# XinMing0411/AC-VAE

Measured on AMD Instinct MI355X. Metric: train-step captions/s (and audio-sec/s) at B=32, 1/2/4/8 MI355X, higher is better.
Workload: dtype f32

## Files before the change

### acvae_amd/csrc/conv_wino.hip

```cpp
#include "mfma_tile.h"
#include "../../include/acvae_hip.h"
#include "conv.h"
#include "prof.h"
#include <type_traits>

namespace {
using namespace mfma;

constexpr int WN_THREADS = 256;
constexpr int WN_TILES = 32;
constexpr int WN_TN = 64;
constexpr int WN_SC = 66, WN_SR = 2 * WN_SC, WN_SQ = 276;
constexpr int WN_BCHUNK = 16 * 2 * 64;
constexpr int WN_MAXC = 2048;
#ifndef WN_PRIO_EDGE
#define WN_PRIO_EDGE 3
#endif
#ifndef WN_PF_DIST
#define WN_PF_DIST 64
#endif

constexpr int WN_RAWBUF = 4 * WN_SQ;
constexpr int WN_EX_F4 = 6 * 512;
constexpr int WN_LDS_F4 = WN_EX_F4 + 64;
static_assert(2 * WN_RAWBUF <= WN_LDS_F4 && 2 * WN_RAWBUF + 2 * WN_MAXC / 4 >= WN_LDS_F4, "exchange + sums overlay the window buffers (+ scale / shift)");

__device__ __forceinline__ void wino_tile(int row, int tw_shift, int& tyl, int& tx) {
  const int cell = (int)((0x1c0c081804141000ULL >> (8 * (row >> 2))) & 0xff) + (row & 3);
  if (tw_shift >= 4) {
    tyl = cell >> tw_shift;
    tx = cell & ((1 << tw_shift) - 1);
  } else {
    const int g = cell >> 4, l16 = cell & 15;
    tx = l16 & ((1 << tw_shift) - 1);
    tyl = g + 2 * (l16 >> tw_shift);
  }
}
__host__ __device__ __forceinline__ int wino_row_pitch(int tw_shift) {
  return tw_shift == 3 ? 12 : tw_shift == 2 ? 6 : (1 << tw_shift) + 1;
}

struct WinoParams {
  const float* X;
  const float* scale;
  const float* shift;
  const float* U;
  float* Y;
  float* partials;
  const float* rY;
  const float* rscale;
  const float* rshift;
  const float* rmean;
  const float* rinvstd;
  int N, H, W, C, Cout;
  int tw_shift;
  int R;
  int bpc;
  int w_shift;
  unsigned bpc_magic;
  int nn_shift;
  int bn_group;
};
__device__ __forceinline__ void wino_tile_of(const WinoParams& p, int t, int nm, int nn, int& bm, int& bn) {
  if (p.bn_group) {
    const int G = p.bn_group, per = nm * G;
    int grp = (int)__fdividef((float)t, (float)per);
    int rem = t - grp * per;
    if (rem < 0) { --grp; rem += per; } else if (rem >= per) { ++grp; rem -= per; }
    bm = rem >> (G >> 1);
    bn = grp * G + (rem & (G - 1));
  } else if (p.nn_shift >= 0) { bn = t & (nn - 1); bm = t >> p.nn_shift; }
  else { bn = t % nn; bm = t / nn; }
}
__device__ __forceinline__ int wino_xcd_tile(const WinoParams& p, int nm, int nn, int& bm, int& bn) {
  const int total = nm * nn;
  const int b = blockIdx.x + blockIdx.y * nm;
  const int q = total >> 3, r = total & 7;
  const int xcd = b & 7, idx = b >> 3;
  const int t = xcd * q + (xcd < r ? xcd : r) + idx;
  wino_tile_of(p, t, nm, nn, bm, bn);
  return t;
}

typedef float f32x2 __attribute__((ext_vector_type(2)));
#define WN_PK_SUB(d, a, b) "v_pk_add_f32 " d ", " a ", " b " neg_lo:[0,1] neg_hi:[0,1]\n\t"
#define WN_PK_ADD(d, a, b) "v_pk_add_f32 " d ", " a ", " b "\n\t"
__device__ __forceinline__ float4 f4sub(float4 a, float4 b) {
  f32x2 lo, hi;
  asm(WN_PK_SUB("%0", "%2", "%4") WN_PK_SUB("%1", "%3", "%5")
      : "=&v"(lo), "=&v"(hi) : "v"(f32x2{a.x, a.y}), "v"(f32x2{a.z, a.w}), "v"(f32x2{b.x, b.y}), "v"(f32x2{b.z, b.w}));
  return make_float4(lo[0], lo[1], hi[0], hi[1]);
}
__device__ __forceinline__ float4 f4add(float4 a, float4 b) {
  f32x2 lo, hi;
  asm(WN_PK_ADD("%0", "%2", "%4") WN_PK_ADD("%1", "%3", "%5")
      : "=&v"(lo), "=&v"(hi) : "v"(f32x2{a.x, a.y}), "v"(f32x2{a.z, a.w}), "v"(f32x2{b.x, b.y}), "v"(f32x2{b.z, b.w}));
  return make_float4(lo[0], lo[1], hi[0], hi[1]);
}
__device__ __forceinline__ void wino_htrans(const float4 (&t)[4], float4 (&v)[4]) {
  f32x2 o[8];
  asm(WN_PK_SUB("%0", "%8", "%12") WN_PK_SUB("%1", "%9", "%13")
      WN_PK_ADD("%2", "%10", "%12") WN_PK_ADD("%3", "%11", "%13")
      WN_PK_SUB("%4", "%12", "%10") WN_PK_SUB("%5", "%13", "%11")
      WN_PK_SUB("%6", "%10", "%14") WN_PK_SUB("%7", "%11", "%15")
      "s_nop 1"
      : "=&v"(o[0]), "=&v"(o[1]), "=&v"(o[2]), "=&v"(o[3]), "=&v"(o[4]), "=&v"(o[5]), "=&v"(o[6]), "=&v"(o[7])
      : "v"(f32x2{t[0].x, t[0].y}), "v"(f32x2{t[0].z, t[0].w}), "v"(f32x2{t[1].x, t[1].y}), "v"(f32x2{t[1].z, t[1].w}),
        "v"(f32x2{t[2].x, t[2].y}), "v"(f32x2{t[2].z, t[2].w}), "v"(f32x2{t[3].x, t[3].y}), "v"(f32x2{t[3].z, t[3].w}));
#pragma unroll
  for (int k = 0; k < 4; ++k) v[k] = make_float4(o[2 * k][0], o[2 * k][1], o[2 * k + 1][0], o[2 * k + 1][1]);
}
__device__ __forceinline__ void pk_sub_ip(float4& a, const float4& b) {
  f32x2 lo{a.x, a.y}, hi{a.z, a.w};
  asm(WN_PK_SUB("%0", "%0", "%2") WN_PK_SUB("%1", "%1", "%3") : "+v"(lo), "+v"(hi) : "v"(f32x2{b.x, b.y}), "v"(f32x2{b.z, b.w}));
  a = make_float4(lo[0], lo[1], hi[0], hi[1]);
}
__device__ __forceinline__ void pk_add_ip(float4& a, const float4& b) {
  f32x2 lo{a.x, a.y}, hi{a.z, a.w};
  asm(WN_PK_ADD("%0", "%0", "%2") WN_PK_ADD("%1", "%1", "%3") : "+v"(lo), "+v"(hi) : "v"(f32x2{b.x, b.y}), "v"(f32x2{b.z, b.w}));
  a = make_float4(lo[0], lo[1], hi[0], hi[1]);
}
__device__ __forceinline__ void wino_htrans_ip(float4 (&t)[4], float4 (&v)[4]) {
  f32x2 a0{t[0].x, t[0].y}, a1{t[0].z, t[0].w}, c0{t[2].x, t[2].y}, c1{t[2].z, t[2].w}, e0{t[3].x, t[3].y}, e1{t[3].z, t[3].w};
  f32x2 n0, n1;
  asm(WN_PK_SUB("%0", "%0", "%2") WN_PK_SUB("%1", "%1", "%3")
      WN_PK_ADD("%6", "%8", "%2") WN_PK_ADD("%7", "%9", "%3")
      WN_PK_SUB("%2", "%2", "%8") WN_PK_SUB("%3", "%3", "%9")
      WN_PK_SUB("%4", "%8", "%4") WN_PK_SUB("%5", "%9", "%5")
      "s_nop 1"
      : "+v"(a0), "+v"(a1), "+v"(c0), "+v"(c1), "+v"(e0), "+v"(e1), "=&v"(n0), "=&v"(n1)
      : "v"(f32x2{t[1].x, t[1].y}), "v"(f32x2{t[1].z, t[1].w}));
  v[0] = make_float4(a0[0], a0[1], a1[0], a1[1]);
  v[1] = make_float4(n0[0], n0[1], n1[0], n1[1]);
  v[2] = make_float4(c0[0], c0[1], c1[0], c1[1]);
  v[3] = make_float4(e0[0], e0[1], e1[0], e1[1]);
}
__device__ __forceinline__ void mfma4_first(f32x16& c, float4 a, float4 b) {
  const f32x16 z = {0.f, 0.f, 0.f, 0.f, 0.f, 0.f, 0.f, 0.f, 0.f, 0.f, 0.f, 0.f, 0.f, 0.f, 0.f, 0.f};
  c = __builtin_amdgcn_mfma_f32_32x32x2f32(a.x, b.x, z, 0, 0, 0);
  c = __builtin_amdgcn_mfma_f32_32x32x2f32(a.y, b.y, c, 0, 0, 0);
  c = __builtin_amdgcn_mfma_f32_32x32x2f32(a.z, b.z, c, 0, 0, 0);
  c = __builtin_amdgcn_mfma_f32_32x32x2f32(a.w, b.w, c, 0, 0, 0);
}
__device__ __forceinline__ void mfma4(f32x16& c, float4 a, float4 b) {
  c = __builtin_amdgcn_mfma_f32_32x32x2f32(a.x, b.x, c, 0, 0, 0);
  c = __builtin_amdgcn_mfma_f32_32x32x2f32(a.y, b.y, c, 0, 0, 0);
  c = __builtin_amdgcn_mfma_f32_32x32x2f32(a.z, b.z, c, 0, 0, 0);
  c = __builtin_amdgcn_mfma_f32_32x32x2f32(a.w, b.w, c, 0, 0, 0);
}

template <int XI, int MODE>
__device__ __forceinline__ void wino_epilogue(const WinoParams& p, const f32x16 (&acc)[8], float2* ex, float* red, int li, int h,
                                              int lane, int n, int ty0, int bm, int bn) {
  constexpr int ROW = XI >> 1, NH = XI & 1;
  constexpr int SET_OTHER = XI == 0 ? 0 : XI == 1 ? 1 : XI == 2 ? 4 : 5;
  constexpr int SET_OWN = XI == 1 ? 2 : XI == 2 ? 3 : -1;
  constexpr int SET_A = XI == 0 ? 1 : XI == 1 ? 0 : XI == 2 ? 1 : 2, SET_B = XI == 0 ? 3 : XI == 1 ? 4 : XI == 2 ? 5 : 4;
  constexpr bool STATS = MODE != 0;
  const int tid = XI * 64 + lane;
  const int H = p.H, W = p.W, Cout = p.Cout;
  const int cout = bn * WN_TN + NH * 32 + li;
  int yk[4], voff[4];
#pragma unroll
  for (int k = 0; k < 4; ++k) {
    int tyl, tx;
    wino_tile(8 * k + 4 * h, p.tw_shift, tyl, tx);
    yk[k] = 2 * (ty0 + tyl) + ROW;
    voff[k] = ((yk[k] * W + 2 * tx) * Cout + cout) * 4;
  }
  int dyj[4], soff[4];
#pragma unroll
  for (int j = 0; j < 4; ++j) {
    dyj[j] = p.tw_shift == 1 ? 4 * (j >> 1) : 0;
    const int dx = p.tw_shift == 1 ? 2 * (j & 1) : 2 * j;
    soff[j] = (dyj[j] * W + dx) * Cout * 4;
  }
  const int pix = Cout * 4;
  float2 yv[MODE == 2 ? 16 : 1];
  float rsc = 0.f, rsh = 0.f, rmu = 0.f, ris = 0.f;
  if (MODE == 2) {
    const __amdgpu_buffer_rsrc_t rrs = __builtin_amdgcn_make_buffer_rsrc(const_cast<float*>(p.rY) + (long)n * H * W * Cout, 0, H * W * Cout * 4, 0x00020000);
#pragma unroll
    for (int r = 0; r < 16; ++r) {
      yv[r].x = __uint_as_float(__builtin_amdgcn_raw_buffer_load_b32(rrs, voff[r >> 2], soff[r & 3], 0));
      yv[r].y = __uint_as_float(__builtin_amdgcn_raw_buffer_load_b32(rrs, voff[r >> 2], soff[r & 3] + pix, 0));
    }
    rsc = p.rscale[cout]; rsh = p.rshift[cout]; rmu = p.rmean[cout]; ris = p.rinvstd[cout];
  }
  float2 keep[16];
#pragma unroll
  for (int r = 0; r < 16; ++r) {
#pragma unroll
    for (int nh = 0; nh < 2; ++nh) {
      const float m0 = acc[0 + nh][r], m1 = acc[2 + nh][r], m2 = acc[4 + nh][r], m3 = acc[6 + nh][r];
      const float2 f = make_float2(m0 + m1 + m2, m1 - m2 - m3);
      if (nh == NH) {
        keep[r] = f;
        if (SET_OWN >= 0) ex[(SET_OWN * 16 + r) * 64 + lane] = f;
      } else {
        ex[(SET_OTHER * 16 + r) * 64 + lane] = f;
      }
    }
  }
  __syncthreads();
  const __amdgpu_buffer_rsrc_t yrs = __builtin_amdgcn_make_buffer_rsrc(p.Y + (long)n * H * W * Cout, 0, H * W * Cout * 4, 0x00020000);
  float s = 0.f, qq = 0.f;
#pragma unroll
  for (int r = 0; r < 16; ++r) {
    const int k = r >> 2, j = r & 3;
    const float2 a = ex[(SET_A * 16 + r) * 64 + lane], b = ex[(SET_B * 16 + r) * 64 + lane];
    const float o0 = ROW ? a.x - (b.x + keep[r].x) : (keep[r].x + a.x) + b.x, o1 = ROW ? a.y - (b.y + keep[r].y) : (keep[r].y + a.y) + b.y;
    __builtin_amdgcn_raw_buffer_store_b32(__float_as_uint(o0), yrs, voff[k], soff[j], 0);
    __builtin_amdgcn_raw_buffer_store_b32(__float_as_uint(o1), yrs, voff[k], soff[j] + pix, 0);
    if (MODE == 1) {
      const bool ok = yk[k] + dyj[j] < H;
      const float a0 = ok ? o0 : 0.f, a1 = ok ? o1 : 0.f;
      s += a0 + a1;
      qq += a0 * a0 + a1 * a1;
    }
    if (MODE == 2) {
      const bool ok = yk[k] + dyj[j] < H;
      const float g0 = (ok && yv[r].x * rsc + rsh > 0.f) ? o0 : 0.f, g1 = (ok && yv[r].y * rsc + rsh > 0.f) ? o1 : 0.f;
      s += g0; s += g1;
      qq += g0 * ((yv[r].x - rmu) * ris); qq += g1 * ((yv[r].y - rmu) * ris);
    }
  }
  if (STATS && p.partials) {
    s += __shfl_xor(s, 32, 64);
    qq += __shfl_xor(qq, 32, 64);
    if (h == 0) {
      red[(ROW * 2 + 0) * 64 + NH * 32 + li] = s;
      red[(ROW * 2 + 1) * 64 + NH * 32 + li] = qq;
    }
    __syncthreads();
    if (tid < WN_TN) {
      const float ts = red[(0 * 2 + 0) * 64 + tid] + red[(1 * 2 + 0) * 64 + tid], tq = red[(0 * 2 + 1) * 64 + tid] + red[(1 * 2 + 1) * 64 + tid];
      float* out = p.partials + (long)bm * 2 * p.Cout + bn * WN_TN + tid;
      out[0] = ts;
      out[p.Cout] = tq;
    }
  }
}

template <int XI, bool ACT, int STATS>
__device__ __forceinline__ void conv_wino_body(const WinoParams& p, float4* raw0, float4* raw1, float4* scsh) {
  __builtin_amdgcn_s_setprio(WN_PRIO_EDGE);
  const int tid = threadIdx.x, lane = tid & 63;
  const int li = lane & 31, h = lane >> 5;
  int bm, bn;
  const int tpos = wino_xcd_tile(p, gridDim.x, gridDim.y, bm, bn);
  const int RW = wino_row_pitch(p.tw_shift), R = p.R;
  const int n = p.bpc == 1 ? bm : (int)__umulhi((unsigned)bm, p.bpc_magic), ty0 = (bm - n * p.bpc) * R;
  const int H = p.H, W = p.W, C = p.C;

  const int nitems = ((2 * R + 2) << p.w_shift) * 4;
  const int q = tid & 3;
  for (int i = tid; i < (2 * R + 2) * 8; i += WN_THREADS) {
    const int ry = i >> 3, side = (i >> 2) & 1, qi = i & 3;
    const int rx = side ? W + 1 : 0;
    const int slot = qi * WN_SQ + (ry & 1) * WN_SR + (rx & 1) * WN_SC + (ry >> 1) * RW + (rx >> 1);
    raw0[slot] = make_float4(0.f, 0.f, 0.f, 0.f);
    raw1[slot] = make_float4(0.f, 0.f, 0.f, 0.f);
  }
  unsigned goff[4];
  int loff[4];
#pragma unroll
  for (int j = 0; j < 4; ++j) {
    const int e = tid + WN_THREADS * j;
    const bool lv = e < nitems;
    const int px = e >> 2;
    const int ry = px >> p.w_shift, x = px & (W - 1), rx = x + 1;
    const int y = 2 * ty0 - 1 + ry;
    const bool ok = lv && y >= 0 && y < H;
    goff[j] = ok ? (unsigned)((((long)(n * H + y) * W + x) * C) + q * 4) : 0u;
    const int slot = q * WN_SQ + (ry & 1) * WN_SR + (rx & 1) * WN_SC + (ry >> 1) * RW + (rx >> 1);
    if (lv && !ok) {
      raw0[slot] = make_float4(0.f, 0.f, 0.f, 0.f);
      raw1[slot] = make_float4(0.f, 0.f, 0.f, 0.f);
    }
    loff[j] = ok ? slot : WN_RAWBUF - 1 - (tid & 7);
  }
  float4 pv[4];
  auto issue_raw = [&](int st) {
#pragma unroll
    for (int j = 0; j < 4; ++j) pv[j] = *reinterpret_cast<const float4*>(p.X + goff[j] + st * 16);
  };
  auto stage_scsh = [&]() {
    if (ACT) {
      for (int i = tid; i < (C >> 2); i += WN_THREADS) {
        scsh[i] = *reinterpret_cast<const float4*>(p.scale + 4 * i);
        scsh[(C >> 2) + i] = *reinterpret_cast<const float4*>(p.shift + 4 * i);
      }
      __syncthreads();
    }
  };
  float4 sc = make_float4(1.f, 1.f, 1.f, 1.f), sh = make_float4(0.f, 0.f, 0.f, 0.f);
  auto read_scsh = [&](int st) {
    if (ACT) {
      sc = scsh[st * 4 + q];
      sh = scsh[(C >> 2) + st * 4 + q];
    }
  };
  auto put_raw_part = [&](float4* raw, int j0) {
#pragma unroll
    for (int j = j0; j < j0 + 2; ++j) {
      float4 v = pv[j];
      if (ACT) {
        v.x = fmaxf(v.x * sc.x + sh.x, 0.f); v.y = fmaxf(v.y * sc.y + sh.y, 0.f);
        v.z = fmaxf(v.z * sc.z + sh.z, 0.f); v.w = fmaxf(v.w * sc.w + sh.w, 0.f);
      }
      raw[loff[j]] = v;
    }
  };
  auto put_raw = [&](float4* raw) { put_raw_part(raw, 0); put_raw_part(raw, 2); };
  const int nchunk = C >> 3;
  const __amdgpu_buffer_rsrc_t urs = __builtin_amdgcn_make_buffer_rsrc(
      const_cast<float*>(p.U + ((long)bn * nchunk) * (WN_BCHUNK * 4)), 0, 0x7fffffff, 0x00020000);
  int tyl_a, tx_a;
  wino_tile(li, p.tw_shift, tyl_a, tx_a);
  const int abase = tyl_a * RW + tx_a;
  constexpr int RA = XI == 0 ? 0 : XI == 2 ? 2 : 1, RB = XI == 0 ? 2 : XI == 1 ? 2 : XI == 2 ? 1 : 3;
  const int rowa = (RA & 1) * WN_SR + (RA >> 1) * RW + abase, rowb = (RB & 1) * WN_SR + (RB >> 1) * RW + abase;
  const int bvoff = (h * 64 + li) * 16;
  auto load_b = [&](int c, int g) {
    typedef unsigned wn_v4u __attribute__((ext_vector_type(4)));
    const wn_v4u v = __builtin_amdgcn_raw_buffer_load_b128(urs, bvoff, c * (WN_BCHUNK * 16) + (XI * 4 + (g >> 1)) * 2048 + (g & 1) * 512, 0);
    return make_float4(__uint_as_float(v.x), __uint_as_float(v.y), __uint_as_float(v.z), __uint_as_float(v.w));
  };

  f32x16 acc[8];

  const int nstage = C >> 4;
  const float4* const aq0 = raw0 + h * WN_SQ;
  const float4* const aq1 = raw1 + h * WN_SQ;
  float4 va[4], vb[4], B[4];
  auto read_row = [&](const float4* rq, int row, float4 (&d)[4]) {
#pragma unroll
    for (int j = 0; j < 4; ++j) d[j] = rq[row + (j & 1) * WN_SC + (j >> 1)];
  };
  auto vertical = [&](float4 (&da)[4], float4 (&db)[4]) {
#pragma unroll
    for (int j = 0; j < 4; ++j) {
      if (XI == 1) pk_add_ip(da[j], db[j]); else pk_sub_ip(da[j], db[j]);
    }
  };

#pragma unroll
  for (int g = 0; g < 4; ++g) B[g] = load_b(0, g);
  issue_raw(0);
  stage_scsh();
  read_scsh(0);
  put_raw(raw0);
  issue_raw(nstage > 1 ? 1 : 0);
  __syncthreads();
  {
    float4 da[4], db[4];
    read_row(aq0, rowa, da);
    read_row(aq0, rowb, db);
    vertical(da, db);
    wino_htrans_ip(da, va);
  }
#define WN_SB() __builtin_amdgcn_sched_barrier(0)
  auto step = [&](int c, auto kk, auto first) {
    constexpr int K = decltype(kk)::value;
    constexpr bool FIRST = decltype(first)::value;
    auto mm = [&](f32x16& a_, float4 x_, float4 y_) { if (FIRST) mfma4_first(a_, x_, y_); else mfma4(a_, x_, y_); };
    constexpr int sub = K & 1, sp = K >> 1;
    float4 (&vc)[4] = sub ? vb : va;
    float4 (&vn)[4] = sub ? va : vb;
    const int st = c >> 1;
    float4* const rnxt = sp ? raw0 : raw1;
    const float4* const nq = sub ? (sp ? aq0 : aq1) : (sp ? aq1 : aq0) + 2 * WN_SQ;
    const int cn = c + 1 < nchunk ? c + 1 : c;
    float4 da[4], db[4];
    const int st1 = st + 1 < nstage ? st + 1 : nstage - 1, st2 = st + 2 < nstage ? st + 2 : nstage - 1;
    if (sub == 0) read_scsh(st1);
    WN_SB();
    mm(acc[0], vc[0], B[0]);
    WN_SB();
    B[0] = load_b(c, 4);
    if (sub == 0) put_raw_part(rnxt, 0);
    WN_SB();
    mm(acc[1], vc[0], B[1]);
    WN_SB();
    B[1] = load_b(c, 5);
    if (sub == 0) put_raw_part(rnxt, 2);
    WN_SB();
    mm(acc[2], vc[1], B[2]);
    WN_SB();
    B[2] = load_b(c, 6);
    if (sub == 0) issue_raw(st2);
    WN_SB();
    mm(acc[3], vc[1], B[3]);
    WN_SB();
    B[3] = load_b(c, 7);
    read_row(nq, rowa, da);
    WN_SB();
    mm(acc[4], vc[2], B[0]);
    WN_SB();
    B[0] = load_b(cn, 0);
    read_row(nq, rowb, db);
    WN_SB();
    mm(acc[5], vc[2], B[1]);
    WN_SB();
    B[1] = load_b(cn, 1);
    WN_SB();
    mm(acc[6], vc[3], B[2]);
    WN_SB();
    B[2] = load_b(cn, 2);
    vertical(da, db);
    WN_SB();
    mm(acc[7], vc[3], B[3]);
    WN_SB();
    B[3] = load_b(cn, 3);
    wino_htrans_ip(da, vn);
    WN_SB();
    if (sub == 0) __syncthreads();
  };
#undef WN_SB
  using std::integral_constant;
  using std::false_type;
  __builtin_amdgcn_s_setprio(0);
  step(0, integral_constant<int, 0>(), std::true_type());
  step(1, integral_constant<int, 1>(), false_type());
  if (2 < nchunk) {
    step(2, integral_constant<int, 2>(), false_type());
    step(3, integral_constant<int, 3>(), false_type());
  }
  for (int c = 4; c < nchunk; c += 4) {
    step(c, integral_constant<int, 0>(), false_type());
    step(c + 1, integral_constant<int, 1>(), false_type());
    if (c + 2 < nchunk) {
      step(c + 2, integral_constant<int, 2>(), false_type());
      step(c + 3, integral_constant<int, 3>(), false_type());
    }
  }
  __builtin_amdgcn_s_setprio(WN_PRIO_EDGE);
  __syncthreads();
  const int lane_e = (int)__builtin_amdgcn_mbcnt_hi(~0u, __builtin_amdgcn_mbcnt_lo(~0u, 0u));
  const int li_e = lane_e & 31, h_e = lane_e >> 5;
  const int tid_e = XI * 64 + lane_e;

  float pfv = 0.f;
  if (!ACT) {
    const int nn_ = (int)gridDim.y;
    const int t2 = tpos + WN_PF_DIST * ((int)gridDim.x * nn_ >= 8 * WN_PF_DIST ? 1 : 0);
    int bm2 = bm, bn2 = bn;
    if (t2 < (int)gridDim.x * nn_) wino_tile_of(p, t2, (int)gridDim.x, nn_, bm2, bn2);
    const int n2 = p.bpc == 1 ? bm2 : (int)__umulhi((unsigned)bm2, p.bpc_magic), ty2 = (bm2 - n2 * p.bpc) * R;
    const int ry = tid_e >> p.w_shift, x = tid_e & (W - 1);
    const int y = 2 * ty2 - 1 + ry;
    if (bm2 < (int)gridDim.x && bm2 != bm && ry < 2 * R + 2 && y >= 0 && y < H)
      pfv = p.X[((long)(n2 * H + y) * W + x) * C];
  }

  float2* exb = reinterpret_cast<float2*>(raw0);
  wino_epilogue<XI, STATS>(p, acc, exb, reinterpret_cast<float*>(raw0 + WN_EX_F4),
                           li_e, h_e, lane_e, n, ty0, bm, bn);
  if (!ACT) asm volatile("" :: "v"(pfv));
}

template <bool ACT, int STATS>
__device__ __forceinline__ void conv_wino_entry(const WinoParams& p, float4* raw, float4* scsh) {
  switch (threadIdx.x >> 6) {
    case 0: conv_wino_body<0, ACT, STATS>(p, raw, raw + WN_RAWBUF, scsh); break;
    case 1: conv_wino_body<1, ACT, STATS>(p, raw, raw + WN_RAWBUF, scsh); break;
    case 2: conv_wino_body<2, ACT, STATS>(p, raw, raw + WN_RAWBUF, scsh); break;
    default: conv_wino_body<3, ACT, STATS>(p, raw, raw + WN_RAWBUF, scsh); break;
  }
}
__global__ __launch_bounds__(WN_THREADS, 2) void conv_wino_kernel(WinoParams p) {
  __shared__ float4 raw[WN_LDS_F4];
  conv_wino_entry<false, 0>(p, raw, nullptr);
}
__global__ __launch_bounds__(WN_THREADS, 2) void conv_wino_bnred_kernel(WinoParams p) {
  __shared__ float4 raw[WN_LDS_F4];
  conv_wino_entry<false, 2>(p, raw, nullptr);
}
__global__ __launch_bounds__(WN_THREADS, 2) void conv_wino_stats_kernel(WinoParams p) {
  __shared__ float4 raw[WN_LDS_F4];
  conv_wino_entry<false, 1>(p, raw, nullptr);
}
__global__ __launch_bounds__(WN_THREADS, 2) void conv_wino_act_kernel(WinoParams p) {
  __shared__ float4 raw[2 * WN_RAWBUF + 2 * WN_MAXC / 4];
  conv_wino_entry<true, 1>(p, raw, raw + 2 * WN_RAWBUF);
}

__device__ __forceinline__ void wino_weights_item(const float* __restrict__ Wt, float4* __restrict__ U, int Cout, int Cin, int dgrad,
                                                  long idx) {
  const int K = dgrad ? Cout : Cin, NO = dgrad ? Cin : Cout;
  {
    const int out = (int)(idx % NO), kq = (int)(idx / NO);
    float u[16][4];
#pragma unroll
    for (int jj = 0; jj < 4; ++jj) {
      const int in = kq * 4 + jj;
      double g[3][3];
#pragma unroll
      for (int a = 0; a < 3; ++a)
#pragma unroll
        for (int b = 0; b < 3; ++b)
          g[a][b] = dgrad ? (double)Wt[((long)in * Cin + out) * 9 + (2 - a) * 3 + (2 - b)]
                          : (double)Wt[((long)out * Cin + in) * 9 + a * 3 + b];
      double t[4][3];
#pragma unroll
      for (int b = 0; b < 3; ++b) {
        t[0][b] = g[0][b];
        t[1][b] = 0.5 * (g[0][b] + g[1][b] + g[2][b]);
        t[2][b] = 0.5 * (g[0][b] - g[1][b] + g[2][b]);
        t[3][b] = g[2][b];
      }
#pragma unroll
      for (int xi = 0; xi < 4; ++xi) {
        u[xi * 4 + 0][jj] = (float)t[xi][0];
        u[xi * 4 + 1][jj] = (float)(0.5 * (t[xi][0] + t[xi][1] + t[xi][2]));
        u[xi * 4 + 2][jj] = (float)(0.5 * (t[xi][0] - t[xi][1] + t[xi][2]));
        u[xi * 4 + 3][jj] = (float)t[xi][2];
      }
    }
    const int cb = out >> 6, col = out & 63, chunk = kq >> 1, hh = kq & 1;
    float4* dst = U + (((long)cb * (K >> 3) + chunk) * 16 * 2 + hh) * 64 + col;
#pragma unroll
    for (int pos = 0; pos < 16; ++pos) dst[(long)pos * 128] = make_float4(u[pos][0], u[pos][1], u[pos][2], u[pos][3]);
  }
}
__global__ void wino_weights_kernel(const float* __restrict__ Wt, float4* __restrict__ U, int Cout, int Cin, int dgrad) {
  const int K = dgrad ? Cout : Cin, NO = dgrad ? Cin : Cout;
  const long total = (long)NO * (K >> 2);
  for (long idx = blockIdx.x * (long)blockDim.x + threadIdx.x; idx < total; idx += (long)gridDim.x * blockDim.x)
    wino_weights_item(Wt, U, Cout, Cin, dgrad, idx);
}
__global__ void wino_weights_batch_kernel(acvae::WinoWeightsBatch b) {
  const long total = b.start[b.n];
  for (long idx = blockIdx.x * (long)blockDim.x + threadIdx.x; idx < total; idx += (long)gridDim.x * blockDim.x) {
    const int l = b.find(idx);
    const acvae::WinoWeightsJob& j = b.job[l];
    wino_weights_item(j.W, reinterpret_cast<float4*>(j.U), j.Cout, j.Cin, j.dgrad, idx - b.start[l]);
  }
}

inline int tile_rows_per_block(int W) { return WN_TILES / (W / 2); }
}

namespace acvae {

bool conv3x3_wino_ok(int H, int W, int Cin, int Cout) {
  if (H < 1 || W < 4 || W > 64 || (W & (W - 1)) != 0) return false;
  return Cin % 16 == 0 && Cin <= WN_MAXC && Cout % WN_TN == 0;
}
long conv3x3_wino_weight_floats(int Cin, int Cout) { return 16L * Cin * Cout; }
int conv_wino_partials_rows(int N, int H, int W) { return N * cdiv(cdiv(H, 2), tile_rows_per_block(W)); }

int conv3x3_wino_weights(const float* W_oihw, float* U, int Cout, int Cin, bool dgrad, hipStream_t st) {
  if (!W_oihw || !U) return ACVAE_EINVAL;
  const int K = dgrad ? Cout : Cin, NO = dgrad ? Cin : Cout;
  if (K % 16 != 0 || NO % WN_TN != 0) return ACVAE_EUNSUPPORTED;
  const long total = (long)NO * (K / 4);
  hipLaunchKernelGGL(wino_weights_kernel, dim3(cdiv(total, 256) > 4096 ? 4096 : cdiv(total, 256)), dim3(256), 0, st, W_oihw,
                     reinterpret_cast<float4*>(U), Cout, Cin, dgrad ? 1 : 0);
  ACVAE_LAUNCH_CHECK();
  return ACVAE_OK;
}

int conv3x3_wino_weights_batch(WinoWeightsBatch& b, hipStream_t st) {
  if (!b.ok()) return ACVAE_EINVAL;
  if (b.n <= 0) return ACVAE_OK;
  for (int l = 0; l < b.n; ++l) {
    const WinoWeightsJob& j = b.job[l];
    if (!j.W || !j.U) return ACVAE_EINVAL;
    const int K = j.dgrad ? j.Cout : j.Cin, NO = j.dgrad ? j.Cin : j.Cout;
    if (K % 16 != 0 || NO % WN_TN != 0) return ACVAE_EUNSUPPORTED;
  }
  const long total = b.seal([](const WinoWeightsJob& j) { return (long)j.Cout * j.Cin / 4; });
  hipLaunchKernelGGL(wino_weights_batch_kernel, dim3(cdiv(total, 256) > 8192 ? 8192 : cdiv(total, 256)), dim3(256), 0, st, b);
  ACVAE_LAUNCH_CHECK();
  return ACVAE_OK;
}

int conv3x3_wino(const float* X, const float* scale, const float* shift, const float* U, float* Y, float* partials, int N,
                 int H, int W, int Cin, int Cout, hipStream_t st, const WinoBnReduce* red) {
  if (!X || !U || !Y) return ACVAE_EINVAL;
  if (red && (scale || !partials || !red->Y || !red->scale || !red->shift || !red->mean || !red->invstd)) return ACVAE_EINVAL;
  if (!conv3x3_wino_ok(H, W, Cin, Cout)) return ACVAE_EUNSUPPORTED;
  if ((long)N * H * W * Cin >= (1L << 32)) return ACVAE_EUNSUPPORTED;
  if (!aligned16(X) || !aligned16(U) || !aligned16(Y) || (scale && (!aligned16(scale) || !aligned16(shift)))) return ACVAE_EALIGN;
  WinoParams p;
  p.X = X; p.scale = scale; p.shift = shift; p.U = U; p.Y = Y; p.partials = partials;
  p.rY = red ? red->Y : nullptr; p.rscale = red ? red->scale : nullptr; p.rshift = red ? red->shift : nullptr;
  p.rmean = red ? red->mean : nullptr; p.rinvstd = red ? red->invstd : nullptr;
  p.N = N; p.H = H; p.W = W; p.C = Cin; p.Cout = Cout;
  const int TW = W / 2;
  p.tw_shift = __builtin_ctz(TW);
  p.R = WN_TILES / TW;
  p.bpc = cdiv(cdiv(H, 2), p.R);
  p.w_shift = p.tw_shift + 1;
  p.bpc_magic = (unsigned)((0x100000000ULL + (unsigned)p.bpc - 1) / (unsigned)p.bpc);
  const int nn = Cout / WN_TN;
  p.nn_shift = (nn & (nn - 1)) == 0 ? __builtin_ctz(nn) : -1;
  {
    int G = 1;
    while (G < 4 && (long)(2 * G) * 4096 * Cin <= (2L << 20)) G *= 2;
    p.bn_group = (G < nn && nn % G == 0 && (long)nn * 4096 * Cin > (2L << 20) && (long)N * p.bpc * nn < (1L << 23)) ? G : 0;
  }
  if ((long)N * p.bpc >= (1L << 20)) return ACVAE_EUNSUPPORTED;
  const dim3 grid(N * p.bpc, Cout / WN_TN);
  prof_begin(ACVAE_PROF_CONV_IGEMM, st);
  if (red) hipLaunchKernelGGL(conv_wino_bnred_kernel, grid, dim3(WN_THREADS), 0, st, p);
  else if (scale) hipLaunchKernelGGL(conv_wino_act_kernel, grid, dim3(WN_THREADS), 0, st, p);
  else if (partials) hipLaunchKernelGGL(conv_wino_stats_kernel, grid, dim3(WN_THREADS), 0, st, p);
  else hipLaunchKernelGGL(conv_wino_kernel, grid, dim3(WN_THREADS), 0, st, p);
  prof_end(ACVAE_PROF_CONV_IGEMM, st);
  ACVAE_LAUNCH_CHECK();
  return ACVAE_OK;
}

}

namespace {
using namespace mfma;
constexpr int WG_XW_PIX = 136;
constexpr int WG_XW_WORDS = WG_XW_PIX * 64;
constexpr int WG_DY_WORDS = 16 * 4 * 64;

struct WinoWgradParams {
  const float* dY;
  const float* X;
  const float* scale;
  const float* shift;
  float* slab;
  int N, H, W, Cin, Cout;
  int st_shift;
  int RS;
  int segs;
  int spc;
  int total;
  int per;
};

template <int XI, int SS>
__device__ __forceinline__ void wino_wgrad_body(const WinoWgradParams& p, float* xw0, float* xw1, float* dy0, float* dy1) {
  const int tid = threadIdx.x, lane = tid & 63, wave = tid >> 6;
  const int li = lane & 31, kh = lane >> 5;
  const int wave_s = __builtin_amdgcn_readfirstlane(wave);
  const int ah = wave >> 2;
  const int z = blockIdx.x, cib = blockIdx.y, cob = blockIdx.z;
  const int H = p.H, W = p.W;
  constexpr int STW = 1 << SS, WC = 2 * STW + 2;
  const int WR = 2 * p.RS + 2;
  const int g_begin = z * p.per, g_end = min(p.total, g_begin + p.per);

  const int quad = tid & 15;
  int xyx[5], xlo[5];
  unsigned xlive = 0;
#pragma unroll
  for (int j = 0; j < 5; ++j) {
    const int e = tid + 512 * j, wp = e >> 4;
    const bool lv = wp < WR * WC;
    xlive |= (lv ? 1u : 0u) << j;
    const int wy = wp / WC, wx = wp - wy * WC;
    xyx[j] = (wy << 8) | wx;
    xlo[j] = wp * 64 + ((quad * 4) ^ (32 * ((wx >> 1) & 1)));
  }
  float4 sc = make_float4(1.f, 1.f, 1.f, 1.f), sh = make_float4(0.f, 0.f, 0.f, 0.f);
  const bool act = p.scale != nullptr;
  if (act) {
    sc = *reinterpret_cast<const float4*>(p.scale + cib * 64 + quad * 4);
    sh = *reinterpret_cast<const float4*>(p.shift + cib * 64 + quad * 4);
  }
  const int WCin = W * p.Cin;
  float4 px[5];
  unsigned xok = 0;
  const int seg_shift = p.segs == 2 ? 1 : 0;
  auto issue_dy = [&](int n, int s, float* dys) {
    const int trow = s >> seg_shift, seg = s & (p.segs - 1);
    const int ty0 = trow * p.RS, tx0 = seg * 16;
#pragma unroll
    for (int i = 0; i < 2; ++i) {
      const int t = wave * 2 + i, pp = lane >> 4, pq = lane & 15;
      const int y = 2 * (ty0 + (t >> p.st_shift)) + (pp >> 1), x = 2 * (tx0 + (t & (STW - 1))) + (pp & 1);
      float* dst = dys + t * 256;
      if (y < H) {
        const float* src = p.dY + (unsigned)(((n * H + y) * W + x) * p.Cout + cob * 64 + ((pq ^ (8 * (t & 1))) << 2));
        __builtin_amdgcn_global_load_lds(src, dst, 16, 0, 0);
      } else {
        *reinterpret_cast<float4*>(dst + lane * 4) = make_float4(0.f, 0.f, 0.f, 0.f);
      }
    }
  };
  auto issue_x = [&](int n, int s) {
    const int trow = s >> seg_shift, seg = s & (p.segs - 1);
    const int ty0 = trow * p.RS, tx0 = seg * 16;
    const int xbase = ((n * H + 2 * ty0 - 1) * W + (2 * tx0 - 1)) * p.Cin + cib * 64 + quad * 4;
    xok = 0;
#pragma unroll
    for (int j = 0; j < 5; ++j) {
      const int wy = xyx[j] >> 8, wx = xyx[j] & 255;
      const int y = 2 * ty0 - 1 + wy, x = 2 * tx0 - 1 + wx;
      const bool ok = ((xlive >> j) & 1u) && y >= 0 && y < H && x >= 0 && x < W;
      xok |= (ok ? 1u : 0u) << j;
      const unsigned off = ok ? (unsigned)(xbase + wy * WCin + wx * p.Cin) : 0u;
      px[j] = *reinterpret_cast<const float4*>(p.X + off);
    }
  };
  auto put_part = [&](float* xw, int j0, int j1) {
#pragma unroll
    for (int j = j0; j < j1; ++j) {
      float4 v = px[j];
      if (act) {
        v.x = fmaxf(v.x * sc.x + sh.x, 0.f); v.y = fmaxf(v.y * sc.y + sh.y, 0.f);
        v.z = fmaxf(v.z * sc.z + sh.z, 0.f); v.w = fmaxf(v.w * sc.w + sh.w, 0.f);
      }
      if (!((xok >> j) & 1u)) v = make_float4(0.f, 0.f, 0.f, 0.f);
      if ((xlive >> j) & 1u) *reinterpret_cast<float4*>(xw + xlo[j]) = v;
    }
  };

  const int ci = ah * 32 + li;
  const int xo01 = kh * 128 + (ci ^ (32 * kh)), xo23 = kh * 128 + (ci ^ (32 * (1 - kh)));
  constexpr int rowstride = WC * 64;
  const int bbase0 = kh * 256 + (li ^ (32 * kh)), bbase1 = kh * 256 + ((32 + li) ^ (32 * kh));
  constexpr int RA = XI == 0 ? 0 : 1, RB = XI == 0 ? 2 : XI == 3 ? 3 : 2;

  f32x16 acc[8];
#pragma unroll
  for (int i = 0; i < 8; ++i)
#pragma unroll
    for (int r = 0; r < 16; ++r) acc[i][r] = 0.f;

  struct Frag { float d[2][4]; float y[2][4]; };
  auto load = [&](auto jj, const float* xw, const float* dys, Frag& f) {
    constexpr int j = decltype(jj)::value;
    constexpr int OFF = ((2 * ((2 * j) >> SS)) * WC + 2 * ((2 * j) & (STW - 1))) * 64;
    const float* x01 = xw + xo01 + OFF;
    const float* x23 = xw + xo23 + OFF;
#pragma unroll
    for (int a = 0; a < 2; ++a) {
      constexpr int ROW[2] = {RA, RB};
      f.d[a][0] = x01[ROW[a] * rowstride + 0 * 64];
      f.d[a][1] = x01[ROW[a] * rowstride + 1 * 64];
      f.d[a][2] = x23[ROW[a] * rowstride + 2 * 64];
      f.d[a][3] = x23[ROW[a] * rowstride + 3 * 64];
    }
    const float* ya = dys + bbase0 + j * 512;
    const float* yb = dys + bbase1 + j * 512;
    f.y[0][0] = ya[0]; f.y[0][1] = ya[64]; f.y[0][2] = ya[128]; f.y[0][3] = ya[192];
    f.y[1][0] = yb[0]; f.y[1][1] = yb[64]; f.y[1][2] = yb[128]; f.y[1][3] = yb[192];
  };
#define WG_A01(D, TL, TH) "v_pk_add_f32 " D ", " TL ", " TH " op_sel_hi:[1,0] neg_lo:[0,1] neg_hi:[0,0]\n\t"
#define WG_A23(D, TL, TH) "v_pk_add_f32 " D ", " TH ", " TL " op_sel:[0,1] op_sel_hi:[1,1] neg_lo:[0,1] neg_hi:[0,1]\n\t"
#define WG_B12(D, R) "v_pk_add_f32 " D ", " R ", " R " op_sel:[0,1] op_sel_hi:[0,1] neg_lo:[0,0] neg_hi:[0,1]\n\t"
#define WG_SUB(D, A, B) "v_pk_add_f32 " D ", " A ", " B " neg_lo:[0,1] neg_hi:[0,1]\n\t"
#define WG_ADD(D, A, B) "v_pk_add_f32 " D ", " A ", " B "\n\t"
  auto mm = [&](const Frag& f) {
    f32x2 a01, a23, b12a, b12b, ra, rb;
    f32x2 tl = {f.d[0][0], f.d[0][1]}, th = {f.d[0][2], f.d[0][3]};
    const f32x2 ul = {f.d[1][0], f.d[1][1]}, uh = {f.d[1][2], f.d[1][3]};
    const f32x2 y0a = {f.y[0][0], f.y[0][1]}, y1a = {f.y[0][2], f.y[0][3]}, y0b = {f.y[1][0], f.y[1][1]}, y1b = {f.y[1][2], f.y[1][3]};
    if constexpr (XI == 0) {
      asm(WG_SUB("%4", "%4", "%6") WG_SUB("%5", "%5", "%7")
          WG_A01("%0", "%4", "%5") WG_A23("%1", "%4", "%5") WG_B12("%2", "%8") WG_B12("%3", "%9") "s_nop 1"
          : "=&v"(a01), "=&v"(a23), "=&v"(b12a), "=&v"(b12b), "+v"(tl), "+v"(th) : "v"(ul), "v"(uh), "v"(y0a), "v"(y0b));
      ra = y0a; rb = y0b;
    } else if constexpr (XI == 3) {
      asm(WG_SUB("%4", "%6", "%4") WG_SUB("%5", "%7", "%5")
          WG_A01("%0", "%4", "%5") WG_A23("%1", "%4", "%5") WG_B12("%2", "%8") WG_B12("%3", "%9") "s_nop 1"
          : "=&v"(a01), "=&v"(a23), "=&v"(b12a), "=&v"(b12b), "+v"(tl), "+v"(th) : "v"(ul), "v"(uh), "v"(y1a), "v"(y1b));
      ra = y1a; rb = y1b;
    } else if constexpr (XI == 1) {
      asm(WG_ADD("%6", "%6", "%8") WG_ADD("%7", "%7", "%9") WG_ADD("%4", "%10", "%11") WG_ADD("%5", "%12", "%13")
          WG_A01("%0", "%6", "%7") WG_A23("%1", "%6", "%7") WG_B12("%2", "%4") WG_B12("%3", "%5") "s_nop 1"
          : "=&v"(a01), "=&v"(a23), "=&v"(b12a), "=&v"(b12b), "=&v"(ra), "=&v"(rb), "+v"(tl), "+v"(th)
          : "v"(ul), "v"(uh), "v"(y0a), "v"(y1a), "v"(y0b), "v"(y1b));
    } else {
      asm(WG_SUB("%6", "%8", "%6") WG_SUB("%7", "%9", "%7") WG_SUB("%4", "%10", "%11") WG_SUB("%5", "%12", "%13")
          WG_A01("%0", "%6", "%7") WG_A23("%1", "%6", "%7") WG_B12("%2", "%4") WG_B12("%3", "%5") "s_nop 1"
          : "=&v"(a01), "=&v"(a23), "=&v"(b12a), "=&v"(b12b), "=&v"(ra), "=&v"(rb), "+v"(tl), "+v"(th)
          : "v"(ul), "v"(uh), "v"(y0a), "v"(y1a), "v"(y0b), "v"(y1b));
    }
    acc[0] = __builtin_amdgcn_mfma_f32_32x32x2f32(a01[0], ra[0], acc[0], 0, 0, 0);
    acc[1] = __builtin_amdgcn_mfma_f32_32x32x2f32(a01[0], rb[0], acc[1], 0, 0, 0);
    acc[2] = __builtin_amdgcn_mfma_f32_32x32x2f32(a01[1], b12a[0], acc[2], 0, 0, 0);
    acc[3] = __builtin_amdgcn_mfma_f32_32x32x2f32(a01[1], b12b[0], acc[3], 0, 0, 0);
    acc[4] = __builtin_amdgcn_mfma_f32_32x32x2f32(a23[0], b12a[1], acc[4], 0, 0, 0);
    acc[5] = __builtin_amdgcn_mfma_f32_32x32x2f32(a23[0], b12b[1], acc[5], 0, 0, 0);
    acc[6] = __builtin_amdgcn_mfma_f32_32x32x2f32(a23[1], ra[1], acc[6], 0, 0, 0);
    acc[7] = __builtin_amdgcn_mfma_f32_32x32x2f32(a23[1], rb[1], acc[7], 0, 0, 0);
  };
#undef WG_A01
#undef WG_A23
#undef WG_B12
#undef WG_SUB
#undef WG_ADD
#define WG_SB() __builtin_amdgcn_sched_barrier(0)
  auto compute = [&](const float* xw, const float* dys, bool more, int nn, int ns, float* xw_n, float* dy_n) {
    Frag fa, fb;
    load(std::integral_constant<int, 0>(), xw, dys, fa);
    load(std::integral_constant<int, 1>(), xw, dys, fb); WG_SB(); mm(fa); WG_SB();
    if (more) issue_dy(nn, ns, dy_n);
    WG_SB();
    load(std::integral_constant<int, 2>(), xw, dys, fa); WG_SB(); mm(fb); WG_SB();
    if (more) issue_x(nn, ns);
    WG_SB();
    load(std::integral_constant<int, 3>(), xw, dys, fb); WG_SB(); mm(fa); WG_SB();
    load(std::integral_constant<int, 4>(), xw, dys, fa); WG_SB(); mm(fb); WG_SB();
    load(std::integral_constant<int, 5>(), xw, dys, fb); WG_SB(); mm(fa); WG_SB();
    if (more) put_part(xw_n, 0, 2);
    WG_SB();
    load(std::integral_constant<int, 6>(), xw, dys, fa); WG_SB(); mm(fb); WG_SB();
    if (more) put_part(xw_n, 2, 4);
    WG_SB();
    load(std::integral_constant<int, 7>(), xw, dys, fb); WG_SB(); mm(fa); WG_SB();
    if (more) put_part(xw_n, 4, 5);
    WG_SB();
    mm(fb);
    WG_SB();
    asm volatile("s_waitcnt vmcnt(0)" ::: "memory");
    __syncthreads();
  };
#undef WG_SB

  if (g_begin < g_end) {
    int n = g_begin / p.spc, sidx = g_begin - n * p.spc;
    issue_dy(n, sidx, dy0);
    issue_x(n, sidx);
    put_part(xw0, 0, 5);
    asm volatile("s_waitcnt vmcnt(0)" ::: "memory");
    __syncthreads();
    for (int g = g_begin; g < g_end; g += 2) {
      if (++sidx == p.spc) { sidx = 0; ++n; }
      compute(xw0, dy0, g + 1 < g_end, n, sidx, xw1, dy1);
      if (g + 1 < g_end) {
        if (++sidx == p.spc) { sidx = 0; ++n; }
        compute(xw1, dy1, g + 2 < g_end, n, sidx, xw0, dy0);
      }
    }
  }

  const int lane_e = (int)__builtin_amdgcn_mbcnt_hi(~0u, __builtin_amdgcn_mbcnt_lo(~0u, 0u));
  const int li_e = lane_e & 31, kh_e = lane_e >> 5;
  const int ah_e = wave_s >> 2;
#pragma unroll
  for (int q = 0; q < 8; ++q) {
    const int pos = XI * 4 + (q >> 1);
    float* out = p.slab + (((long)z * 16 + pos) * p.Cin + cib * 64 + ah_e * 32) * p.Cout + cob * 64 + (q & 1) * 32 + li_e;
#pragma unroll
    for (int r = 0; r < 16; ++r) {
      const int row = (r & 3) + 8 * (r >> 2) + 4 * kh_e;
      out[(long)row * p.Cout] = acc[q][r];
    }
  }
}

template <int SS>
__device__ __forceinline__ void wino_wgrad_entry(const WinoWgradParams& p, float* xw0, float* xw1, float* dy0, float* dy1) {
  switch ((threadIdx.x >> 6) & 3) {
    case 0: wino_wgrad_body<0, SS>(p, xw0, xw1, dy0, dy1); break;
    case 1: wino_wgrad_body<1, SS>(p, xw0, xw1, dy0, dy1); break;
    case 2: wino_wgrad_body<2, SS>(p, xw0, xw1, dy0, dy1); break;
    default: wino_wgrad_body<3, SS>(p, xw0, xw1, dy0, dy1); break;
  }
}
#define WINO_WGRAD_KERNEL(SS)                                                                                    \
  __global__ __launch_bounds__(512) void conv_wino_wgrad_kernel_s##SS(WinoWgradParams p) {                     \
    __shared__ float xw0[WG_XW_WORDS], xw1[WG_XW_WORDS];                                                         \
    __shared__ float dy0[WG_DY_WORDS], dy1[WG_DY_WORDS];                                                         \
    wino_wgrad_entry<SS>(p, xw0, xw1, dy0, dy1);                                                                 \
  }
WINO_WGRAD_KERNEL(1) WINO_WGRAD_KERNEL(2) WINO_WGRAD_KERNEL(3) WINO_WGRAD_KERNEL(4)
#undef WINO_WGRAD_KERNEL

template <int PAIRS>
__global__ __launch_bounds__(256) void wino_wgrad_reduce_kernel(const float* __restrict__ slab, float* __restrict__ dW, int Z, int Cout,
                                                                int Cin) {
  constexpr int PG = 256 / PAIRS;
  constexpr int PPT = 16 / PG;
  __shared__ float su[16][PAIRS];
  const long total = (long)Cin * Cout, per_z = 16 * total;
  const int lp = threadIdx.x % PAIRS, pg = threadIdx.x / PAIRS;
  const long pair = (long)blockIdx.x * PAIRS + lp;
  if (pair < total) {
#pragma unroll
    for (int k = 0; k < PPT; ++k) {
      const int pos = pg * PPT + k;
      const long idx = (long)pos * total + pair;
      double s0 = 0.0, s1 = 0.0, s2 = 0.0, s3 = 0.0;
      int z = 0;
      for (; z + 4 <= Z; z += 4) {
        const float a = slab[(long)z * per_z + idx], b = slab[(long)(z + 1) * per_z + idx];
        const float c = slab[(long)(z + 2) * per_z + idx], d = slab[(long)(z + 3) * per_z + idx];
        s0 += (double)a; s1 += (double)b; s2 += (double)c; s3 += (double)d;
      }
      for (; z < Z; ++z) s0 += (double)slab[(long)z * per_z + idx];
      su[pos][lp] = (float)((s0 + s1) + (s2 + s3));
    }
  }
  __syncthreads();
  if (pg != 0 || pair >= total) return;
  const int co = (int)(pair % Cout), ci = (int)(pair / Cout);
  double u[16];
#pragma unroll
  for (int pos = 0; pos < 16; ++pos) u[pos] = (double)su[pos][lp];
  double t[3][4];
#pragma unroll
  for (int nu = 0; nu < 4; ++nu) {
    t[0][nu] = u[0 * 4 + nu] + 0.5 * (u[1 * 4 + nu] + u[2 * 4 + nu]);
    t[1][nu] = 0.5 * (u[1 * 4 + nu] - u[2 * 4 + nu]);
    t[2][nu] = 0.5 * (u[1 * 4 + nu] + u[2 * 4 + nu]) + u[3 * 4 + nu];
  }
  float* out = dW + ((long)co * Cin + ci) * 9;
#pragma unroll
  for (int a = 0; a < 3; ++a) {
    out[a * 3 + 0] = (float)(t[a][0] + 0.5 * (t[a][1] + t[a][2]));
    out[a * 3 + 1] = (float)(0.5 * (t[a][1] - t[a][2]));
    out[a * 3 + 2] = (float)(0.5 * (t[a][1] + t[a][2]) + t[a][3]);
  }
}

struct WgradPlan { int st_shift, RS, segs, spc, total, Z, per; };
inline WgradPlan wino_wgrad_plan(int N, int H, int W, int Cin, int Cout) {
  WgradPlan g;
  const int TW = W / 2, TH = (H + 1) / 2;
  const int STW = TW < 16 ? TW : 16;
  g.st_shift = __builtin_ctz(STW);
  g.RS = 16 / STW;
  g.segs = TW / STW;
  g.spc = TW >= 16 ? TH * g.segs : (TH + g.RS - 1) / g.RS;
  g.total = N * g.spc;
  const int blocks = (Cin / 64) * (Cout / 64);
  int Z = 256 / blocks;
  if (Z < 1) Z = 1;
  if (Z > g.total) Z = g.total;
  g.per = (g.total + Z - 1) / Z;
  g.Z = (g.total + g.per - 1) / g.per;
  return g;
}
}

namespace acvae {
bool conv3x3_wino_wgrad_ok(int H, int W, int Cin, int Cout) {
  if (H < 1 || W < 4 || W > 64 || (W & (W - 1)) != 0) return false;
  return Cin % 64 == 0 && Cout % 64 == 0;
}
static bool wino_wgrad_fits(int N, int H, int W, int Cin, int Cout) {
  return (long)N * H * W * (Cin > Cout ? Cin : Cout) < (1L << 31);
}
long conv3x3_wino_wgrad_slab_floats(int N, int H, int W, int Cin, int Cout) {
  if (!conv3x3_wino_wgrad_ok(H, W, Cin, Cout)) return 0;
  return (long)wino_wgrad_plan(N, H, W, Cin, Cout).Z * 16 * Cin * Cout;
}
int conv3x3_wino_wgrad(const float* dY, const float* X, const float* scale, const float* shift, float* dW_oihw, float* slab,
                       int N, int H, int W, int Cin, int Cout, hipStream_t st) {
  if (!dY || !X || !dW_oihw || !slab) return ACVAE_EINVAL;
  if (!conv3x3_wino_wgrad_ok(H, W, Cin, Cout) || !wino_wgrad_fits(N, H, W, Cin, Cout)) return ACVAE_EUNSUPPORTED;
  if (!aligned16(dY) || !aligned16(X) || !aligned16(slab) || (scale && (!aligned16(scale) || !aligned16(shift)))) return ACVAE_EALIGN;
  const WgradPlan g = wino_wgrad_plan(N, H, W, Cin, Cout);
  WinoWgradParams p;
  p.dY = dY; p.X = X; p.scale = scale; p.shift = shift; p.slab = slab;
  p.N = N; p.H = H; p.W = W; p.Cin = Cin; p.Cout = Cout;
  p.st_shift = g.st_shift; p.RS = g.RS; p.segs = g.segs; p.spc = g.spc; p.total = g.total; p.per = g.per;
  prof_begin(ACVAE_PROF_CONV_WGRAD, st);
  const dim3 wgrid(g.Z, Cin / 64, Cout / 64);
  switch (g.st_shift) {
    case 1: hipLaunchKernelGGL(conv_wino_wgrad_kernel_s1, wgrid, dim3(512), 0, st, p); break;
    case 2: hipLaunchKernelGGL(conv_wino_wgrad_kernel_s2, wgrid, dim3(512), 0, st, p); break;
    case 3: hipLaunchKernelGGL(conv_wino_wgrad_kernel_s3, wgrid, dim3(512), 0, st, p); break;
    default: hipLaunchKernelGGL(conv_wino_wgrad_kernel_s4, wgrid, dim3(512), 0, st, p); break;
  }
  prof_end(ACVAE_PROF_CONV_WGRAD, st);
  const long total = (long)Cin * Cout;
  if (total < 16 * 1024)
    hipLaunchKernelGGL(wino_wgrad_reduce_kernel<16>, dim3((unsigned)cdiv(total, 16)), dim3(256), 0, st, slab, dW_oihw, g.Z, Cout, Cin);
  else
    hipLaunchKernelGGL(wino_wgrad_reduce_kernel<64>, dim3((unsigned)cdiv(total, 64)), dim3(256), 0, st, slab, dW_oihw, g.Z, Cout, Cin);
  ACVAE_LAUNCH_CHECK();
  return ACVAE_OK;
}
}
```

Before: 2084.

## Specialize Winograd wgrad on activation flag and use buffer loads for input tiles

Templates the Winograd weight-gradient kernel on a compile-time ACT flag and makes the tile geometry constexpr per SS, so the loop trip counts and live masks become static. Input tile loads now go through buffer resource loads, where an out-of-range offset returns zero, which replaces the per-element bounds-checked address arithmetic. dY offsets are precomputed per thread, and the BN+ReLU masking is folded into fmed3. The LDS window grows to 160 pixels so unused slots can be written without guards, at the cost of more shared memory per block and possibly lower occupancy.

After: 2109 (median of 6 runs). 1.01x the previous value.

```diff
diff --git a/acvae_amd/csrc/conv_wino.hip b/acvae_amd/csrc/conv_wino.hip
--- a/acvae_amd/csrc/conv_wino.hip
+++ b/acvae_amd/csrc/conv_wino.hip
@@ -618,7 +618,7 @@
 
 namespace {
 using namespace mfma;
-constexpr int WG_XW_PIX = 136;
+constexpr int WG_XW_PIX = 160;
 constexpr int WG_XW_WORDS = WG_XW_PIX * 64;
 constexpr int WG_DY_WORDS = 16 * 4 * 64;
 
@@ -637,7 +637,7 @@
   int per;
 };
 
-template <int XI, int SS>
+template <int XI, int SS, bool ACT>
 __device__ __forceinline__ void wino_wgrad_body(const WinoWgradParams& p, float* xw0, float* xw1, float* dy0, float* dy1) {
   const int tid = threadIdx.x, lane = tid & 63, wave = tid >> 6;
   const int li = lane & 31, kh = lane >> 5;
@@ -646,42 +646,49 @@
   const int z = blockIdx.x, cib = blockIdx.y, cob = blockIdx.z;
   const int H = p.H, W = p.W;
   constexpr int STW = 1 << SS, WC = 2 * STW + 2;
-  const int WR = 2 * p.RS + 2;
+  constexpr int RS = 16 >> SS, WR = 2 * RS + 2;
+  constexpr int NPIX = WR * WC;
+  constexpr int NIT = (NPIX * 16 + 511) / 512;
+  static_assert(NIT * 32 <= WG_XW_PIX, "window of a stage and the slots past it");
   const int g_begin = z * p.per, g_end = min(p.total, g_begin + p.per);
 
   const int quad = tid & 15;
-  int xyx[5], xlo[5];
-  unsigned xlive = 0;
-#pragma unroll
-  for (int j = 0; j < 5; ++j) {
-    const int e = tid + 512 * j, wp = e >> 4;
-    const bool lv = wp < WR * WC;
-    xlive |= (lv ? 1u : 0u) << j;
+  const int xlo = (tid >> 4) * 64 + ((quad * 4) ^ (32 * ((tid >> 5) & 1)));
+  int xr[NIT], xo[NIT], xcb = 0;
+#pragma unroll
+  for (int j = 0; j < NIT; ++j) {
+    const int wp = (tid + 512 * j) >> 4;
     const int wy = wp / WC, wx = wp - wy * WC;
-    xyx[j] = (wy << 8) | wx;
-    xlo[j] = wp * 64 + ((quad * 4) ^ (32 * ((wx >> 1) & 1)));
+    xo[j] = ((wy * W + wx) * p.Cin + quad * 4) * 4;
+    xr[j] = wp < NPIX && (SS == 4 || (wx >= 1 && wx <= WC - 2)) ? wy : (1 << 22);
+    xcb |= (wx == 0 ? 1 << j : 0) | (wx == WC - 1 ? 1 << (8 + j) : 0);
   }
   float4 sc = make_float4(1.f, 1.f, 1.f, 1.f), sh = make_float4(0.f, 0.f, 0.f, 0.f);
-  const bool act = p.scale != nullptr;
-  if (act) {
+  if (ACT) {
     sc = *reinterpret_cast<const float4*>(p.scale + cib * 64 + quad * 4);
     sh = *reinterpret_cast<const float4*>(p.shift + cib * 64 + quad * 4);
   }
-  const int WCin = W * p.Cin;
-  float4 px[5];
-  unsigned xok = 0;
+  int dyr[2];
+  unsigned dyo[2];
+#pragma unroll
+  for (int i = 0; i < 2; ++i) {
+    const int t = wave * 2 + i, pp = lane >> 4, pq = lane & 15;
+    dyr[i] = 2 * (t >> SS) + (pp >> 1);
+    dyo[i] = (unsigned)(((dyr[i] * W + 2 * (t & (STW - 1)) + (pp & 1)) * p.Cout + ((pq ^ (8 * (t & 1))) << 2)) * 4);
+  }
+  typedef unsigned wg_v4u __attribute__((ext_vector_type(4)));
+  wg_v4u px[NIT];
+  bool xok[NIT];
   const int seg_shift = p.segs == 2 ? 1 : 0;
   auto issue_dy = [&](int n, int s, float* dys) {
     const int trow = s >> seg_shift, seg = s & (p.segs - 1);
-    const int ty0 = trow * p.RS, tx0 = seg * 16;
+    const int ys = 2 * trow * RS;
+    const char* src = reinterpret_cast<const char*>(p.dY + ((long)(n * H + ys) * W + 32 * seg) * p.Cout + cob * 64);
 #pragma unroll
     for (int i = 0; i < 2; ++i) {
-      const int t = wave * 2 + i, pp = lane >> 4, pq = lane & 15;
-      const int y = 2 * (ty0 + (t >> p.st_shift)) + (pp >> 1), x = 2 * (tx0 + (t & (STW - 1))) + (pp & 1);
-      float* dst = dys + t * 256;
-      if (y < H) {
-        const float* src = p.dY + (unsigned)(((n * H + y) * W + x) * p.Cout + cob * 64 + ((pq ^ (8 * (t & 1))) << 2));
-        __builtin_amdgcn_global_load_lds(src, dst, 16, 0, 0);
+      float* dst = dys + (wave * 2 + i) * 256;
+      if (dyr[i] < H - ys) {
+        __builtin_amdgcn_global_load_lds(reinterpret_cast<const float*>(src + dyo[i]), dst, 16, 0, 0);
       } else {
         *reinterpret_cast<float4*>(dst + lane * 4) = make_float4(0.f, 0.f, 0.f, 0.f);
       }
@@ -689,29 +696,32 @@
   };
   auto issue_x = [&](int n, int s) {
     const int trow = s >> seg_shift, seg = s & (p.segs - 1);
-    const int ty0 = trow * p.RS, tx0 = seg * 16;
-    const int xbase = ((n * H + 2 * ty0 - 1) * W + (2 * tx0 - 1)) * p.Cin + cib * 64 + quad * 4;
-    xok = 0;
-#pragma unroll
-    for (int j = 0; j < 5; ++j) {
-      const int wy = xyx[j] >> 8, wx = xyx[j] & 255;
-      const int y = 2 * ty0 - 1 + wy, x = 2 * tx0 - 1 + wx;
-      const bool ok = ((xlive >> j) & 1u) && y >= 0 && y < H && x >= 0 && x < W;
-      xok |= (ok ? 1u : 0u) << j;
-      const unsigned off = ok ? (unsigned)(xbase + wy * WCin + wx * p.Cin) : 0u;
-      px[j] = *reinterpret_cast<const float4*>(p.X + off);
+    const int y0 = 2 * trow * RS - 1, x0 = 32 * seg - 1;
+    const __amdgpu_buffer_rsrc_t xrs = __builtin_amdgcn_make_buffer_rsrc(
+        const_cast<float*>(p.X + ((long)(n * H + y0) * W + x0) * p.Cin + cib * 64), 0, 0x7fffffff, 0x00020000);
+    int xbad = 0;
+    if (SS == 4) {
+      const int b = xcb & ((x0 < 0 ? 0xff : 0) | (x0 + WC - 1 >= W ? 0xff00 : 0));
+      xbad = b | (b >> 8);
+    }
+#pragma unroll
+    for (int j = 0; j < NIT; ++j) {
+      bool ok = (unsigned)(xr[j] + y0) < (unsigned)H;
+      if (SS == 4) ok = ok & !((xbad >> j) & 1);
+      xok[j] = ok;
+      px[j] = __builtin_amdgcn_raw_buffer_load_b128(xrs, ok ? xo[j] : (int)0x80000000, 0, 0);
     }
   };
   auto put_part = [&](float* xw, int j0, int j1) {
 #pragma unroll
-    for (int j = j0; j < j1; ++j) {
-      float4 v = px[j];
-      if (act) {
-        v.x = fmaxf(v.x * sc.x + sh.x, 0.f); v.y = fmaxf(v.y * sc.y + sh.y, 0.f);
-        v.z = fmaxf(v.z * sc.z + sh.z, 0.f); v.w = fmaxf(v.w * sc.w + sh.w, 0.f);
+    for (int j = j0; j < j1 && j < NIT; ++j) {
+      float4 v = make_float4(__uint_as_float(px[j].x), __uint_as_float(px[j].y), __uint_as_float(px[j].z), __uint_as_float(px[j].w));
+      if (ACT) {
+        const float m = xok[j] ? __builtin_inff() : 0.f;
+        v.x = __builtin_amdgcn_fmed3f(v.x * sc.x + sh.x, 0.f, m); v.y = __builtin_amdgcn_fmed3f(v.y * sc.y + sh.y, 0.f, m);
+        v.z = __builtin_amdgcn_fmed3f(v.z * sc.z + sh.z, 0.f, m); v.w = __builtin_amdgcn_fmed3f(v.w * sc.w + sh.w, 0.f, m);
       }
-      if (!((xok >> j) & 1u)) v = make_float4(0.f, 0.f, 0.f, 0.f);
-      if ((xlive >> j) & 1u) *reinterpret_cast<float4*>(xw + xlo[j]) = v;
+      *reinterpret_cast<float4*>(xw + xlo + 2048 * j) = v;
     }
   };
 
@@ -736,10 +746,12 @@
 #pragma unroll
     for (int a = 0; a < 2; ++a) {
       constexpr int ROW[2] = {RA, RB};
-      f.d[a][0] = x01[ROW[a] * rowstride + 0 * 64];
-      f.d[a][1] = x01[ROW[a] * rowstride + 1 * 64];
-      f.d[a][2] = x23[ROW[a] * rowstride + 2 * 64];
-      f.d[a][3] = x23[ROW[a] * rowstride + 3 * 64];
+      const float* xe = (ROW[a] & 1) ? x23 : x01;
+      const float* xf = (ROW[a] & 1) ? x01 : x23;
+      f.d[a][0] = xe[ROW[a] * rowstride + 0 * 64];
+      f.d[a][1] = xe[ROW[a] * rowstride + 1 * 64];
+      f.d[a][2] = xf[ROW[a] * rowstride + 2 * 64];
+      f.d[a][3] = xf[ROW[a] * rowstride + 3 * 64];
     }
     const float* ya = dys + bbase0 + j * 512;
     const float* yb = dys + bbase1 + j * 512;
@@ -851,22 +863,25 @@
   }
 }
 
-template <int SS>
+template <int SS, bool ACT>
 __device__ __forceinline__ void wino_wgrad_entry(const WinoWgradParams& p, float* xw0, float* xw1, float* dy0, float* dy1) {
   switch ((threadIdx.x >> 6) & 3) {
-    case 0: wino_wgrad_body<0, SS>(p, xw0, xw1, dy0, dy1); break;
-    case 1: wino_wgrad_body<1, SS>(p, xw0, xw1, dy0, dy1); break;
-    case 2: wino_wgrad_body<2, SS>(p, xw0, xw1, dy0, dy1); break;
-    default: wino_wgrad_body<3, SS>(p, xw0, xw1, dy0, dy1); break;
-  }
-}
-#define WINO_WGRAD_KERNEL(SS)                                                                                    \
-  __global__ __launch_bounds__(512) void conv_wino_wgrad_kernel_s##SS(WinoWgradParams p) {                     \
+    case 0: wino_wgrad_body<0, SS, ACT>(p, xw0, xw1, dy0, dy1); break;
+    case 1: wino_wgrad_body<1, SS, ACT>(p, xw0, xw1, dy0, dy1); break;
+    case 2: wino_wgrad_body<2, SS, ACT>(p, xw0, xw1, dy0, dy1); break;
+    default: wino_wgrad_body<3, SS, ACT>(p, xw0, xw1, dy0, dy1); break;
+  }
+}
+#define WINO_WGRAD_KERNEL(NAME, SS, ACT)                                                                         \
+  __global__ __launch_bounds__(512) void NAME##SS(WinoWgradParams p) {                                          \
     __shared__ float xw0[WG_XW_WORDS], xw1[WG_XW_WORDS];                                                         \
     __shared__ float dy0[WG_DY_WORDS], dy1[WG_DY_WORDS];                                                         \
-    wino_wgrad_entry<SS>(p, xw0, xw1, dy0, dy1);                                                                 \
-  }
-WINO_WGRAD_KERNEL(1) WINO_WGRAD_KERNEL(2) WINO_WGRAD_KERNEL(3) WINO_WGRAD_KERNEL(4)
+    wino_wgrad_entry<SS, ACT>(p, xw0, xw1, dy0, dy1);                                                            \
+  }
+WINO_WGRAD_KERNEL(conv_wino_wgrad_kernel_s, 1, false) WINO_WGRAD_KERNEL(conv_wino_wgrad_kernel_s, 2, false)
+WINO_WGRAD_KERNEL(conv_wino_wgrad_kernel_s, 3, false) WINO_WGRAD_KERNEL(conv_wino_wgrad_kernel_s, 4, false)
+WINO_WGRAD_KERNEL(conv_wino_wgrad_act_kernel_s, 1, true) WINO_WGRAD_KERNEL(conv_wino_wgrad_act_kernel_s, 2, true)
+WINO_WGRAD_KERNEL(conv_wino_wgrad_act_kernel_s, 3, true) WINO_WGRAD_KERNEL(conv_wino_wgrad_act_kernel_s, 4, true)
 #undef WINO_WGRAD_KERNEL
 
 template <int PAIRS>
@@ -960,11 +975,15 @@
   p.st_shift = g.st_shift; p.RS = g.RS; p.segs = g.segs; p.spc = g.spc; p.total = g.total; p.per = g.per;
   prof_begin(ACVAE_PROF_CONV_WGRAD, st);
   const dim3 wgrid(g.Z, Cin / 64, Cout / 64);
-  switch (g.st_shift) {
-    case 1: hipLaunchKernelGGL(conv_wino_wgrad_kernel_s1, wgrid, dim3(512), 0, st, p); break;
-    case 2: hipLaunchKernelGGL(conv_wino_wgrad_kernel_s2, wgrid, dim3(512), 0, st, p); break;
-    case 3: hipLaunchKernelGGL(conv_wino_wgrad_kernel_s3, wgrid, dim3(512), 0, st, p); break;
-    default: hipLaunchKernelGGL(conv_wino_wgrad_kernel_s4, wgrid, dim3(512), 0, st, p); break;
+  switch (g.st_shift * 2 + (scale ? 1 : 0)) {
+    case 2: hipLaunchKernelGGL(conv_wino_wgrad_kernel_s1, wgrid, dim3(512), 0, st, p); break;
+    case 3: hipLaunchKernelGGL(conv_wino_wgrad_act_kernel_s1, wgrid, dim3(512), 0, st, p); break;
+    case 4: hipLaunchKernelGGL(conv_wino_wgrad_kernel_s2, wgrid, dim3(512), 0, st, p); break;
+    case 5: hipLaunchKernelGGL(conv_wino_wgrad_act_kernel_s2, wgrid, dim3(512), 0, st, p); break;
+    case 6: hipLaunchKernelGGL(conv_wino_wgrad_kernel_s3, wgrid, dim3(512), 0, st, p); break;
+    case 7: hipLaunchKernelGGL(conv_wino_wgrad_act_kernel_s3, wgrid, dim3(512), 0, st, p); break;
+    case 8: hipLaunchKernelGGL(conv_wino_wgrad_kernel_s4, wgrid, dim3(512), 0, st, p); break;
+    default: hipLaunchKernelGGL(conv_wino_wgrad_act_kernel_s4, wgrid, dim3(512), 0, st, p); break;
   }
   prof_end(ACVAE_PROF_CONV_WGRAD, st);
   const long total = (long)Cin * Cout;
```
